# deepreinforce-ai/CUDA-L2

Measured on AMD Instinct MI355X. Metric: HGEMM TFLOP/s, higher is better.
Workload: dtype f16

## Files before the change

cuda-l2_amd/build.py:

```python
from __future__ import annotations

import concurrent.futures as cf
import hashlib
import os
import shutil
import subprocess
import sys
from pathlib import Path

PKG_DIR = Path(__file__).resolve().parent
REPO_DIR = PKG_DIR.parent
CSRC = PKG_DIR / "csrc"
INCLUDE = REPO_DIR / "include"
BUILD = PKG_DIR / "build"
OBJ = BUILD / "obj"
_SUFFIX = os.environ.get("HGEMM_LIB_SUFFIX", "")
LIB_DIR = PKG_DIR / ("lib_" + _SUFFIX if _SUFFIX else "lib")
BIN_DIR = PKG_DIR / "bin"
ROCM = Path(os.environ.get("ROCM_PATH", "/opt/rocm"))
HIPCC = str(ROCM / "bin" / "hipcc")
ARCH = "gfx950"

LIB_SOURCES = [
    "hgemm_inst_g0.hip",
    "hgemm_inst_g1.hip",
    "hgemm_inst_g2.hip",
    "hgemm_inst_g3.hip",
    "hgemm_inst_g4.hip",
    "hgemm_inst_g5.hip",
    "hgemm_inst_g6.hip",
    "hgemm_inst_g7.hip",
    "hgemm_inst_g8.hip",
    "hgemm_inst_g9.hip",
    "hgemm_inst_g10.hip",
    "hgemm_inst_g11.hip",
    "hgemm_inst_g12.hip",
    "hgemm_inst_g13.hip",
    "hgemm_inst_g14.hip",
    "hgemm_inst_g15.hip",
    "hgemm_inst_g16.hip",
    "hgemm_inst_g17.hip",
    "hgemm_registry.hip",
    "hgemm_plan.hip",
    "hgemm_api.hip",
    "hgemm_baselines.hip",
]

HIP_FLAGS = os.environ.get("HGEMM_EXTRA_HIPFLAGS", "").split() + [f"--offload-arch={ARCH}", "-O3", "-std=c++17", "-fPIC", "-Wall", "-Wno-unused-function",
             "-Wno-unused-result", "-Wno-unused-value", "-DROCBLAS_NO_DEPRECATED_WARNINGS", "-D__HIP_PLATFORM_AMD__"]


def _headers_digest() -> str:
    h = hashlib.sha256()
    for d in (CSRC, INCLUDE):
        for p in sorted(d.rglob("*")):
            if p.suffix in (".hpp", ".h", ".def", ".inc"):
                h.update(p.name.encode())
                h.update(p.read_bytes())
    return h.hexdigest()


def _run(cmd: list[str], verbose: bool) -> None:
    if verbose:
        print(" ".join(cmd), flush=True)
    res = subprocess.run(cmd, capture_output=True, text=True)
    if res.returncode != 0:
        sys.stderr.write(res.stdout + res.stderr)
        raise RuntimeError(f"build step failed ({res.returncode}): {' '.join(cmd)}")
    if verbose and (res.stdout or res.stderr):
        print(res.stdout + res.stderr, flush=True)


def compile_object(src: Path, extra_flags: list[str], hdr_digest: str, verbose: bool = False) -> Path:
    OBJ.mkdir(parents=True, exist_ok=True)
    cmd_core = [HIPCC, *HIP_FLAGS, *extra_flags, f"-I{CSRC}", f"-I{INCLUDE}", "-c"]
    key = hashlib.sha256()
    key.update(" ".join(cmd_core).encode())
    key.update(hdr_digest.encode())
    key.update(src.read_bytes())
    obj = OBJ / f"{src.stem}-{key.hexdigest()[:20]}.o"
    if not obj.exists():
        tmp = obj.with_suffix(f".tmp{os.getpid()}.o")
        _run([*cmd_core, str(src), "-o", str(tmp)], verbose)
        os.replace(tmp, obj)
    return obj


def build_library(verbose: bool = False, jobs: int | None = None) -> Path:
    hdr = _headers_digest()
    jobs = jobs or min(8, os.cpu_count() or 1)
    srcs = [CSRC / s for s in LIB_SOURCES]
    with cf.ThreadPoolExecutor(max_workers=jobs) as ex:
        objs = list(ex.map(lambda s: compile_object(s, [], hdr, verbose), srcs))
    LIB_DIR.mkdir(exist_ok=True)
    lib = LIB_DIR / "libhgemm_mi355x.so"
    stamp = LIB_DIR / ".libhgemm_mi355x.stamp"
    want = hashlib.sha256(" ".join(o.name for o in objs).encode()).hexdigest()
    if lib.exists() and stamp.exists() and stamp.read_text() == want:
        return lib
    tmp = lib.with_suffix(f".tmp{os.getpid()}.so")
    _run([HIPCC, f"--offload-arch={ARCH}", "-shared", "-fPIC", *map(str, objs), "-o", str(tmp),
          f"-L{ROCM / 'lib'}", "-lrocblas", "-lhipblaslt", "-lamdhip64",
          "-Wl,--no-undefined", "-Wl,-soname,libhgemm_mi355x.so"], verbose)
    os.replace(tmp, lib)
    stamp.write_text(want)
    return lib


def build_tools(verbose: bool = False) -> list[Path]:
    lib = build_library(verbose)
    hdr = _headers_digest()
    BIN_DIR.mkdir(exist_ok=True)
    out = []
    for name in ("hgemm_tune",):
        src = CSRC / "tools" / f"{name}.cpp"
        if not src.exists():
            continue
        obj = compile_object(src, ["-x", "hip"], hdr, verbose)
        exe = BIN_DIR / name
        stamp = BIN_DIR / f".{name}.stamp"
        want = obj.name + lib.name + str(lib.stat().st_mtime_ns)
        if not (exe.exists() and stamp.exists() and stamp.read_text() == want):
            _run([HIPCC, f"--offload-arch={ARCH}", str(obj), "-o", str(exe), f"-L{LIB_DIR}", "-lhgemm_mi355x",
                  f"-L{ROCM / 'lib'}", "-lamdhip64", "-lrocm_smi64", "-Wl,-rpath,$ORIGIN/../lib", f"-Wl,-rpath,{ROCM / 'lib'}"],
# ... 61 lines not shown
```

cuda-l2_amd/csrc/hgemm_api.hip:

```cpp
#include "hgemm_plan.hpp"
#include "hgemm_kernel_nn.hpp"
#include "hgemm_act.hpp"
#include "../../include/hgemm_mi355x.h"

#include <algorithm>
#include <atomic>
#include <cmath>
#include <cstdint>
#include <cstdlib>
#include <cstring>
#include <mutex>
#include <vector>

using namespace hgemm_mi355x;

namespace {

thread_local int g_last_hip_error = 0;
#ifdef HGEMM_ABLATION
int g_debug_flags = 0;
#endif
#ifdef HGEMM_TIMELINE
unsigned long long* g_timeline = nullptr;
int g_timeline_slots = 0;
// ... 734 lines not shown
  g_ws.clear();
  g_ws_retired.clear();
  return rc;
}

int hgemm_mi355x_release_stream_workspace(void* stream) {
  int dev = 0;
  if (hipGetDevice(&dev) != hipSuccess) return HGEMM_ERR_HIP;
  std::lock_guard<std::mutex> lk(g_ws_mutex);
  for (size_t i = 0; i < g_ws.size(); ++i) {
    if (g_ws[i].device != dev || g_ws[i].stream != (hipStream_t)stream) continue;
    int rc = HGEMM_OK;
    if (g_ws[i].ptr) {
      if (g_ws[i].captured) g_ws_retired.push_back(g_ws[i].ptr);
      else if (hipFree(g_ws[i].ptr) != hipSuccess) rc = HGEMM_ERR_HIP;
    }
    g_ws.erase(g_ws.begin() + (long)i);
    return rc;
  }
  return HGEMM_OK;
}

int hgemm_mi355x_reserve_workspace(int M, int N, int K, void* stream) {
  if (M <= 0 || N <= 0 || K <= 0) return HGEMM_ERR_BAD_ARG;
  int cfg = 0, splits = 1, group = 1;
  const int st = hgemm_mi355x_plan(M, N, K, &cfg, &splits, &group);
  if (st != HGEMM_OK) return st;
  const size_t ws = std::max(hgemm_mi355x_plan_workspace_bytes(cfg, splits, M, N, K), kCounterBytes + (size_t)256 * 256 * 256 * sizeof(float));
  float* slabs = nullptr; unsigned* counters = nullptr;
  const int rc = ensure_workspace(ws - kCounterBytes, (hipStream_t)stream, &slabs, &counters);
  return rc == HGEMM_ERR_NO_WORKSPACE_INTERNAL ? HGEMM_ERR_NO_WORKSPACE : rc;
}

int hgemm_mi355x_launch(int config_id, int splits_arg, int group_m, const void* a, const void* b,
                        const void* b_col_major, void* c, int M, int N, int K, int lda, int ldb,
                        int ldc, void* stream) {
  DisarmTiming disarm_timing;
  if (!a || !c || M <= 0 || N <= 0 || K <= 0) return HGEMM_ERR_BAD_ARG;
  if (config_id >= g_num_kernels || config_id < HGEMM_CONFIG_RAGGED) return HGEMM_ERR_BAD_ARG;
#ifdef HGEMM_TIMELINE
  ++g_timeline_count;
#endif
  hipStream_t s = (hipStream_t)stream;
  const bool aligned = mfma_path_ok(a, b_col_major, c, M, N, K, lda, ldb, ldc);
  unsigned ruled_out = 0;
  auto resolve = [&] {
    return resolve_launch(config_id, splits_arg, group_m, b != nullptr, b_col_major != nullptr, aligned, M, N, K, lda, ldb, ldc, ruled_out);
  };
  LaunchPlan p = resolve();
  float* slabs = nullptr; unsigned* counters = nullptr;
  while (p.status == HGEMM_OK && p.slab_bytes) {
    const int st = ensure_workspace(p.slab_bytes, s, &slabs, &counters);
    if (st == HGEMM_OK) break;
    if (st != HGEMM_ERR_NO_WORKSPACE_INTERNAL && p.form != FORM_HYBRID) return st;
    ruled_out |= 1u << p.form;
    p = resolve();
  }
  if (p.status != HGEMM_OK) return p.status;
  for (int i = 0; i < p.n; ++i) {
    GemmArgs& g = p.d[i].g;
    g.A = (const f16*)a; g.Bt = (const f16*)b_col_major; g.C = (f16*)c;
    if (p.d[i].epi != EPI_C16) {
      g.partial = slabs;
      if (p.counters) g.counters = counters;
    }
    const TimingSlot ts = timing_slot(p.d[i].start, p.d[i].stop);
    switch (p.d[i].thunk) {
      case THUNK_ENTRY: g_kernel_table[config_id].launch(g, p.d[i].grid, s, p.d[i].epi, ts); break;
      case THUNK_SPLITK_REDUCE: launch_splitk_reduce(g.partial, g.C, M, N, ldc, g.splits, s, ts); break;
      case THUNK_TAIL_REDUCE: launch_tail_reduce(g, g_kernel_table[config_id].bm, g_kernel_table[config_id].bn, s, ts); break;
      case THUNK_RAGGED: launch_ragged(g, s, ts); break;
      case THUNK_GENERIC: launch_generic((const f16*)a, (const f16*)b, (f16*)c, M, N, K, lda, N, ldc, s, ts); break;
    }
  }
  hipError_t err = hipGetLastError();
  if (err != hipSuccess) { g_last_hip_error = (int)err; return HGEMM_ERR_HIP; }
  return HGEMM_OK;
}

int hgemm_mi355x_set_one_item_kernel(int on) { return sq_one_set_enabled(on); }

unsigned long long hgemm_mi355x_one_item_kernel_launches(void) { return sq_one_launch_count(); }

int hgemm_mi355x_one_item_kernel_takes(int config_id, int splits, int group_m, int M, int N, int K, int lda, int ldb, int ldc) {
  if (M <= 0 || N <= 0 || K <= 0 || config_id >= g_num_kernels || config_id < HGEMM_CONFIG_RAGGED) return HGEMM_ERR_BAD_ARG;
  const LaunchPlan p = resolve_launch(config_id, splits, group_m, false, true, true, M, N, K, lda, ldb, ldc, 0);
  if (p.status != HGEMM_OK) return p.status;
  static const int q256 = hgemm_mi355x_config_by_name("q256x256_w2x2");
  if (config_id != q256) return 0;
  for (int i = 0; i < p.n; ++i)
    if (p.d[i].thunk == THUNK_ENTRY && sq_one_takes(p.d[i].g, p.d[i].grid, p.d[i].epi)) return 1;
  return 0;
}

int hgemm_mi355x_set_insitu(int enable) {
  const int old = insitu_enabled() ? 1 : 0;
  g_insitu_mode.store(enable ? 1 : 0);
  if (!enable) {
    std::lock_guard<std::mutex> lk(g_insitu_mutex);
    g_insitu.clear();
    g_insitu_epoch.fetch_add(1, std::memory_order_release);
  }
  return old;
}

int hgemm_mi355x_insitu_enabled(void) { return insitu_enabled() ? 1 : 0; }

int hgemm_mi355x_insitu_candidates(int M, int N, int K, int config_id[3], int splits[3], int group_m[3]) {
  if (M <= 0 || N <= 0 || K <= 0 || !config_id || !splits || !group_m) return 0;
  PlanTriple c[3];
  const int n = insitu_candidates(M, N, K, c);
  for (int i = 0; i < n; ++i) { config_id[i] = c[i].cfg; splits[i] = c[i].splits; group_m[i] = c[i].group_m; }
  return n;
}

int hgemm_mi355x_insitu_choice(int M, int N, int K, int* config_id, int* splits, int* group_m) {
  PlanTriple p;
  int dev = 0;
  if (hipGetDevice(&dev) != hipSuccess) { (void)hipGetLastError(); dev = 0; }
  if (!config_id || !splits || !group_m || !insitu_lookup(dev, M, N, K, &p)) return 0;
  *config_id = p.cfg; *splits = p.splits; *group_m = p.group_m;
  return 1;
}

int hgemm_mi355x_fp32(const void* a, const void* b, const void* bt, void* c, int M, int N, int K,
                      void* stream) {
  return run(HGEMM_ACC_FP32, a, b, bt, c, M, N, K, stream);
}

int hgemm_mi355x_fp16(const void* a, const void* b, const void* bt, void* c, int M, int N, int K,
                      void* stream) {
  return run(HGEMM_ACC_FP16, a, b, bt, c, M, N, K, stream);
}

int hgemm_mi355x_nn_num_configs(void) { return kLayoutNN.t.count; }
const char* hgemm_mi355x_nn_config_name(int id) { return tr_config_name(kLayoutNN, id); }
int hgemm_mi355x_nn_config_by_name(const char* name) { return tr_config_by_name(kLayoutNN, name); }
int hgemm_mi355x_nn_config_info(int id, int out[8]) { return tr_config_info(kLayoutNN, id, out); }
int hgemm_mi355x_nn_plan(int M, int N, int K, int* nn_config, int* splits) { return tr_plan(kLayoutNN, M, N, K, nn_config, splits); }
int hgemm_mi355x_nn_runs(int nn_config, int M, int N, int K, int lda, int ldb, int ldc) { return tr_runs(kLayoutNN, TR_F16, kOutC16, nn_config, M, N, K, lda, ldb, ldc); }
size_t hgemm_mi355x_nn_plan_workspace_bytes(int nn_config, int splits, int M, int N, int K) {
  return tr_plan_workspace_bytes(kLayoutNN, nn_config, splits, M, N, K);
}
int hgemm_mi355x_nn_reserve_workspace(int M, int N, int K, void* stream) { return tr_reserve_workspace(kLayoutNN, M, N, K, stream); }
int hgemm_mi355x_launch_nn(int nn_config, int splits_arg, const void* a, const void* b, void* c, int M, int N, int K, int lda, int ldb,
                           int ldc, void* stream) {
  return tr_launch(kLayoutNN, TR_F16, kOutC16, nn_config, splits_arg, a, b, nullptr, c, M, N, K, lda, ldb, ldc, stream);
}
int hgemm_mi355x_nn_fp32(const void* a, const void* b, void* c, int M, int N, int K, void* stream) { return tr_run(kLayoutNN, TR_F16, kOutC16, a, b, nullptr, c, M, N, K, stream); }
int hgemm_mi355x_nn_fp16(const void* a, const void* b, void* c, int M, int N, int K, void* stream) { return tr_run(kLayoutNN, TR_F16, kOutC16, a, b, nullptr, c, M, N, K, stream); }
int hgemm_mi355x_selfcheck_launch_nn(int nn_config, int splits, int operands, int M, int N, int K, int lda, int ldb, int ldc, int ruled_out,
                                     long long out[20]) {
  return tr_selfcheck_launch(kLayoutNN, TR_F16, kOutC16, nn_config, splits, operands, M, N, K, lda, ldb, ldc, ruled_out, out);
}

int hgemm_mi355x_ta_num_configs(void) { return kLayoutTA.t.count; }
const char* hgemm_mi355x_ta_config_name(int id) { return tr_config_name(kLayoutTA, id); }
int hgemm_mi355x_ta_config_by_name(const char* name) { return tr_config_by_name(kLayoutTA, name); }
int hgemm_mi355x_ta_config_info(int id, int out[8]) { return tr_config_info(kLayoutTA, id, out); }
int hgemm_mi355x_ta_plan(int M, int N, int K, int* ta_config, int* splits) { return tr_plan(kLayoutTA, M, N, K, ta_config, splits); }
int hgemm_mi355x_ta_runs(int ta_config, int M, int N, int K, int lda, int ldb, int ldc) { return tr_runs(kLayoutTA, TR_F16, kOutC16, ta_config, M, N, K, lda, ldb, ldc); }
size_t hgemm_mi355x_ta_plan_workspace_bytes(int ta_config, int splits, int M, int N, int K) {
  return tr_plan_workspace_bytes(kLayoutTA, ta_config, splits, M, N, K);
}
int hgemm_mi355x_ta_reserve_workspace(int M, int N, int K, void* stream) { return tr_reserve_workspace(kLayoutTA, M, N, K, stream); }
int hgemm_mi355x_launch_ta(int ta_config, int splits_arg, const void* a_col_major, const void* b, void* c, int M, int N, int K, int lda,
                           int ldb, int ldc, void* stream) {
  return tr_launch(kLayoutTA, TR_F16, kOutC16, ta_config, splits_arg, a_col_major, b, nullptr, c, M, N, K, lda, ldb, ldc, stream);
}
int hgemm_mi355x_ta_fp32(const void* a_col_major, const void* b, void* c, int M, int N, int K, void* stream) { return tr_run(kLayoutTA, TR_F16, kOutC16, a_col_major, b, nullptr, c, M, N, K, stream); }
int hgemm_mi355x_ta_fp16(const void* a_col_major, const void* b, void* c, int M, int N, int K, void* stream) { return tr_run(kLayoutTA, TR_F16, kOutC16, a_col_major, b, nullptr, c, M, N, K, stream); }
int hgemm_mi355x_selfcheck_launch_ta(int ta_config, int splits, int operands, int M, int N, int K, int lda, int ldb, int ldc, int ruled_out,
                                     long long out[20]) {
  return tr_selfcheck_launch(kLayoutTA, TR_F16, kOutC16, ta_config, splits, operands, M, N, K, lda, ldb, ldc, ruled_out, out);
}
// ... 304 lines not shown
```

cuda-l2_amd/csrc/hgemm_inst_g13.hip:

```cpp
#include "hgemm_launch.hpp"
#include "hgemm_kernel_sq_one.hpp"

#include <atomic>

namespace hgemm_mi355x {

template __global__ void hgemm_tn_sq_one_kernel<CfgSQOne>(const GemmArgs);

namespace {
#ifdef HGEMM_TIMELINE
std::atomic<int> g_sq_one_on{0};
#else
std::atomic<int> g_sq_one_on{1};
#endif
std::atomic<unsigned long long> g_sq_one_launches{0};
}

int sq_one_set_enabled(int on) { return g_sq_one_on.exchange(on ? 1 : 0); }
unsigned long long sq_one_launch_count() { return g_sq_one_launches.load(); }

bool sq_one_takes(const GemmArgs& g, int grid, int epi) {
  if (!g_sq_one_on.load(std::memory_order_relaxed)) return false;
  if (epi != EPI_C16 || !c_takes_wide_stores(g)) return false;
  if (g.K % (BK * CfgSQOne::KT) != 0 || g.K / BK < SQ_ONE_MIN_STEPS) return false;
  if (g.splits != 1 || g.tail_tiles != 0 || g.items > grid) return false;
  if (g.flags & (ARG_XCD_STAGGER | ARG_PHASE_OFFSET | ARG_PHASE_OFFSET4)) return false;
#ifdef HGEMM_ABLATION
  if (g.debug) return false;
#endif
  return true;
}

bool launch_sq_one(const GemmArgs& g, int grid, hipStream_t stream, int epi, TimingSlot ts) {
  if (!sq_one_takes(g, grid, epi)) return false;
  g_sq_one_launches.fetch_add(1, std::memory_order_relaxed);
  HGEMM_LAUNCH((hgemm_tn_sq_one_kernel<CfgSQOne>), grid, CfgSQOne::THREADS, stream, ts, g);
  return true;
}

}
```

cuda-l2_amd/csrc/hgemm_launch.hpp:

```cpp
#pragma once
#include "hgemm_kernel_rs.hpp"
#include "hgemm_kernel_sq.hpp"
#include "hgemm_kernel_wd.hpp"
#include "hgemm_kernel_lu.hpp"

#include <hip/hip_ext.h>

#include <type_traits>

namespace hgemm_mi355x {

struct LaunchTiming { hipEvent_t start = nullptr, stop = nullptr; };
extern thread_local LaunchTiming t_launch_timing;

struct TimingSlot { hipEvent_t start = nullptr, stop = nullptr; };
inline TimingSlot timing_slot(bool first, bool last) {
  TimingSlot s;
  if (first) { s.start = t_launch_timing.start; t_launch_timing.start = nullptr; }
  if (last) { s.stop = t_launch_timing.stop; t_launch_timing.stop = nullptr; }
  return s;
}

#define HGEMM_LAUNCH(KERNEL, GRID, THREADS, STREAM, SLOT, ...)                                              \
  do {                                                                                                      \
    if ((SLOT).start || (SLOT).stop)                                                                        \
      hipExtLaunchKernelGGL(KERNEL, dim3(GRID), dim3(THREADS), 0, STREAM, (SLOT).start, (SLOT).stop, 0,     \
                            __VA_ARGS__);                                                                   \
    else                                                                                                    \
      hipLaunchKernelGGL(KERNEL, dim3(GRID), dim3(THREADS), 0, STREAM, __VA_ARGS__);                        \
  } while (0)

template <class CFG>
void launch_cfg(const GemmArgs& g, int grid, hipStream_t stream, int epi, TimingSlot ts) {
  if (epi == EPI_STREAMK) {
    if constexpr (CFG::BM * CFG::BN <= 256 * 128) HGEMM_LAUNCH((hgemm_tn_sk_kernel<CFG>), grid, CFG::THREADS, stream, ts, g);
  } else if (epi == EPI_FUSED)
    HGEMM_LAUNCH((hgemm_tn_kernel<CFG, EPI_FUSED>), grid, CFG::THREADS, stream, ts, g);
  else if (epi == EPI_SLAB)
    HGEMM_LAUNCH((hgemm_tn_kernel<CFG, EPI_SLAB>), grid, CFG::THREADS, stream, ts, g);
  else
    HGEMM_LAUNCH((hgemm_tn_kernel<CFG, EPI_C16>), grid, CFG::THREADS, stream, ts, g);
}

inline bool c_takes_wide_stores(const GemmArgs& g) {
  return ((g.N & 7) == 0) && ((g.ldc & 7) == 0) && ((reinterpret_cast<uintptr_t>(g.C) & 15) == 0);
}

template <class CFG>
void launch_sp(const GemmArgs& g, int grid, hipStream_t stream, int epi, TimingSlot ts) {
  const bool wide = c_takes_wide_stores(g);
  if (epi == EPI_FUSED)
    HGEMM_LAUNCH((hgemm_tn_sp_kernel<CFG, SP_EPI_FUSED>), grid, CFG::THREADS, stream, ts, g);
  else if (epi == EPI_SLAB)
    HGEMM_LAUNCH((hgemm_tn_sp_kernel<CFG, SP_EPI_SLAB>), grid, CFG::THREADS, stream, ts, g);
  else if (wide)
    HGEMM_LAUNCH((hgemm_tn_sp_kernel<CFG, SP_EPI_WIDE>), grid, CFG::THREADS, stream, ts, g);
  else
    HGEMM_LAUNCH((hgemm_tn_sp_kernel<CFG, SP_EPI_NARROW>), grid, CFG::THREADS, stream, ts, g);
}

template <class CFG, int FLAG>
void launch_sq_variant(const GemmArgs& g, int grid, hipStream_t stream, int epi, TimingSlot ts) {
  const bool wide = c_takes_wide_stores(g);
  if (epi == EPI_FUSED)
    HGEMM_LAUNCH((hgemm_tn_sq_kernel<CFG, SP_EPI_FUSED | FLAG>), grid, CFG::THREADS, stream, ts, g);
  else if (epi == EPI_SLAB)
    HGEMM_LAUNCH((hgemm_tn_sq_kernel<CFG, SP_EPI_SLAB | FLAG>), grid, CFG::THREADS, stream, ts, g);
  else if (wide)
    HGEMM_LAUNCH((hgemm_tn_sq_kernel<CFG, SP_EPI_WIDE | FLAG>), grid, CFG::THREADS, stream, ts, g);
  else
    HGEMM_LAUNCH((hgemm_tn_sq_kernel<CFG, SP_EPI_NARROW | FLAG>), grid, CFG::THREADS, stream, ts, g);
}

bool launch_sq_one(const GemmArgs& g, int grid, hipStream_t stream, int epi, TimingSlot ts);
bool sq_one_takes(const GemmArgs& g, int grid, int epi);
int sq_one_set_enabled(int on);
unsigned long long sq_one_launch_count();

template <class CFG>
void launch_sq(const GemmArgs& g, int grid, hipStream_t stream, int epi, TimingSlot ts) {
  if constexpr (std::is_same_v<CFG, CfgSQOne>) {
    if (launch_sq_one(g, grid, stream, epi, ts)) return;
  }
  if constexpr (CFG::MI == 16) {
    if (g.K % (BK * CFG::KT) != 0) return launch_sq_variant<CFG, EPI_KTAIL>(g, grid, stream, epi, ts);
    if (g.flags & ARG_XCD_STAGGER) return launch_sq_variant<CFG, EPI_KSTAGGER>(g, grid, stream, epi, ts);
  }
  launch_sq_variant<CFG, 0>(g, grid, stream, epi, ts);
}

template <class CFG, int FLAG>
void launch_rs_variant(const GemmArgs& g, int grid, hipStream_t stream, int epi, TimingSlot ts) {
  if (epi == EPI_FUSED)
    HGEMM_LAUNCH((hgemm_tn_rs_kernel<CFG, EPI_FUSED | FLAG>), grid, CFG::THREADS, stream, ts, g);
  else if (epi == EPI_SLAB)
    HGEMM_LAUNCH((hgemm_tn_rs_kernel<CFG, EPI_SLAB | FLAG>), grid, CFG::THREADS, stream, ts, g);
  else
    HGEMM_LAUNCH((hgemm_tn_rs_kernel<CFG, EPI_C16 | FLAG>), grid, CFG::THREADS, stream, ts, g);
}

template <class CFG>
void launch_rs(const GemmArgs& g, int grid, hipStream_t stream, int epi, TimingSlot ts) {
  if (epi == EPI_STREAMK)
    HGEMM_LAUNCH((hgemm_tn_rs_sk_kernel<CFG>), grid, CFG::THREADS, stream, ts, g);
  else if (g.K % CFG::BKS != 0)
    launch_rs_variant<CFG, EPI_KTAIL>(g, grid, stream, epi, ts);
  else
    launch_rs_variant<CFG, 0>(g, grid, stream, epi, ts);
}

template <class CFG>
void launch_wd(const GemmArgs& g, int grid, hipStream_t stream, int epi, TimingSlot ts) {
  if (epi == EPI_FUSED)
    HGEMM_LAUNCH((hgemm_tn_wd_kernel<CFG, EPI_FUSED>), grid, CFG::THREADS, stream, ts, g);
  else if (epi == EPI_SLAB)
    HGEMM_LAUNCH((hgemm_tn_wd_kernel<CFG, EPI_SLAB>), grid, CFG::THREADS, stream, ts, g);
  else
    HGEMM_LAUNCH((hgemm_tn_wd_kernel<CFG, EPI_C16>), grid, CFG::THREADS, stream, ts, g);
}

template <class CFG>
void launch_lu(const GemmArgs& g, int grid, hipStream_t stream, int epi, TimingSlot ts) {
  if (epi == EPI_SLAB)
    HGEMM_LAUNCH((hgemm_tn_lu_kernel<CFG, EPI_SLAB>), grid, CFG::THREADS, stream, ts, g);
  else
    HGEMM_LAUNCH((hgemm_tn_lu_kernel<CFG, EPI_C16>), grid, CFG::THREADS, stream, ts, g);
}

enum class Family : char { T = 't', S = 's', Q = 'q', R = 'r', W = 'w', U = 'u' };
enum class KTail : char { NONE, PADDED, DIRECT };

struct KernelEntry {
  const char* name;
  Family family;
  int bm, bn, wm, wn, mi, nbuf;
  int threads, lds_bytes;
  void (*launch)(const GemmArgs&, int, hipStream_t, int, TimingSlot);
  int persistent_wgs;
  bool has_fused;
  int kgran;
  KTail ktail;
  int sk_wgs_per_cu;
  bool explicit_only;
};
inline bool w_splits_k(const KernelEntry& e) { return e.family == Family::W && e.wm * e.wn == 1; }

extern const KernelEntry g_kernel_table[];
extern const int g_num_kernels;

void launch_splitk_reduce(const float* partial, f16* C, int M, int N, int ldc, int splits,
                          hipStream_t stream, TimingSlot ts);
void launch_tail_reduce(const GemmArgs& g, int BM, int BN, hipStream_t stream, TimingSlot ts);
void launch_ragged(const GemmArgs& g, hipStream_t stream, TimingSlot ts);
void launch_generic(const f16* A, const f16* B, f16* C, int M, int N, int K, int lda, int ldb,
                    int ldc, hipStream_t stream, TimingSlot ts);

}
```

include/hgemm_mi355x.h:

```cpp
#ifndef HGEMM_MI355X_H_
#define HGEMM_MI355X_H_

#include <stddef.h>

#ifdef __cplusplus
extern "C" {
#endif

typedef enum {
  HGEMM_OK = 0,
  HGEMM_ERR_BAD_ARG = -1,
  HGEMM_ERR_TOO_LARGE = -2,
  HGEMM_ERR_HIP = -3,
  HGEMM_ERR_BACKEND = -4,
  HGEMM_ERR_NOT_READY = -5,
  HGEMM_ERR_NO_ALGO = -6,
  HGEMM_ERR_NO_WORKSPACE = -7
} hgemm_status_t;

typedef enum { HGEMM_ACC_FP32 = 0, HGEMM_ACC_FP16 = 1 } hgemm_acc_t;

#define HGEMM_CONFIG_GENERIC (-1)
#define HGEMM_CONFIG_RAGGED  (-2)

// ... 97 lines not shown
int bgemm_mi355x_tn_num_configs(void);
const char* bgemm_mi355x_tn_config_name(int tn_config);
int bgemm_mi355x_tn_config_by_name(const char* name);
int bgemm_mi355x_tn_config_info(int tn_config, int out[8]);
int bgemm_mi355x_tn_plan(int M, int N, int K, int* tn_config, int* splits);
size_t bgemm_mi355x_tn_plan_workspace_bytes(int tn_config, int splits, int M, int N, int K);
int bgemm_mi355x_tn_reserve_workspace(int M, int N, int K, void* stream);

int bgemm_mi355x_tn_bias(const void* a, const void* b_col_major, const void* bias, void* c, int M, int N, int K, void* stream);
int bgemm_mi355x_launch_tn_bias(int tn_config, int splits, const void* a, const void* b_col_major, const void* bias, void* c,
                                int M, int N, int K, int lda, int ldb, int ldc, void* stream);
int bgemm_mi355x_tn_bias_runs(int tn_config, int M, int N, int K, int lda, int ldb, int ldc);

#define HGEMM_ACT_RELU 1
#define HGEMM_ACT_GELU 2
#define HGEMM_ACT_GELU_TANH 3
int bgemm_mi355x_tn_bias_act(const void* a, const void* b_col_major, const void* bias, void* c, int M, int N, int K, int act, void* stream);
int bgemm_mi355x_launch_tn_bias_act(int tn_config, int splits, const void* a, const void* b_col_major, const void* bias, void* c,
                                    int M, int N, int K, int lda, int ldb, int ldc, int act, void* stream);
int bgemm_mi355x_tn_bias_act_runs(int tn_config, int M, int N, int K, int lda, int ldb, int ldc);

int bgemm_mi355x_tn_bias_act_aux(const void* a, const void* b_col_major, const void* bias, void* c, void* z_out, int M, int N, int K, int act,
                                 void* stream);
int bgemm_mi355x_launch_tn_bias_act_aux(int tn_config, int splits, const void* a, const void* b_col_major, const void* bias, void* c,
                                        void* z_out, int M, int N, int K, int lda, int ldb, int ldc, int ldz, int act, void* stream);
int bgemm_mi355x_tn_bias_act_aux_runs(int tn_config, int M, int N, int K, int lda, int ldb, int ldc, int ldz);

int bgemm_mi355x_nn_dact(const void* a, const void* b, const void* z, void* c, int M, int N, int K, int act, void* stream);
int bgemm_mi355x_launch_nn_dact(int nn_config, int splits, const void* a, const void* b, const void* z, void* c, int M, int N, int K,
                                int lda, int ldb, int ldc, int ldz, int act, void* stream);
int bgemm_mi355x_nn_dact_runs(int nn_config, int M, int N, int K, int lda, int ldb, int ldc, int ldz);

int bgemm_mi355x_nn_dact_dbias(const void* a, const void* b, const void* z, void* c, float* db32, int M, int N, int K, int act,
                               int accumulate, void* stream);
int bgemm_mi355x_launch_nn_dact_dbias(int nn_config, int splits, const void* a, const void* b, const void* z, void* c, float* db32, int M,
                                      int N, int K, int lda, int ldb, int ldc, int ldz, int act, int accumulate, void* stream);
int bgemm_mi355x_nn_dact_dbias_runs(int nn_config, int M, int N, int K, int lda, int ldb, int ldc, int ldz);
size_t bgemm_mi355x_nn_dact_dbias_plan_workspace_bytes(int nn_config, int splits, int M, int N, int K);
int bgemm_mi355x_nn_dact_dbias_reserve_workspace(int M, int N, int K, void* stream);

int bgemm_mi355x_colsum_c32(const void* x, float* out32, int M, int N, int ldx, int accumulate, void* stream);

const char* hgemm_mi355x_strerror(int status);
int hgemm_mi355x_last_hip_error(void);
const char* hgemm_mi355x_version(void);

int hgemm_rocblas_init(void);
int hgemm_rocblas_destroy(void);
int hgemm_rocblas_nn(const void* a, const void* b, void* c, int M, int N, int K, int acc, void* stream);
int hgemm_rocblas_tn(const void* a, const void* b_col_major, void* c, int M, int N, int K, int acc, void* stream);
int hgemm_rocblas_ta(const void* a_col_major, const void* b, void* c, int M, int N, int K, int acc, void* stream);
int bgemm_rocblas_nn(const void* a, const void* b, void* c, int M, int N, int K, void* stream);
int bgemm_rocblas_ta(const void* a_col_major, const void* b, void* c, int M, int N, int K, void* stream);
int bgemm_rocblas_tn(const void* a, const void* b_col_major, void* c, int M, int N, int K, void* stream);

int hgemm_hipblaslt_heuristic_init(void);
int hgemm_hipblaslt_heuristic_destroy(void);
int hgemm_hipblaslt_heuristic_nn(const void* a, const void* b, void* c, int M, int N, int K, int acc, void* stream);
int hgemm_hipblaslt_heuristic_tn(const void* a, const void* b_col_major, void* c, int M, int N, int K, int acc, void* stream);

int hgemm_hipblaslt_autotune_init(void);
int hgemm_hipblaslt_autotune_destroy(void);
int hgemm_hipblaslt_autotune_find_best_nn(int M, int N, int K, int acc);
int hgemm_hipblaslt_autotune_find_best_tn(int M, int N, int K, int acc);
int hgemm_hipblaslt_autotune_nn(const void* a, const void* b, void* c, int M, int N, int K, int acc, void* stream);
int hgemm_hipblaslt_autotune_tn(const void* a, const void* b_col_major, void* c, int M, int N, int K, int acc, void* stream);
int hgemm_hipblaslt_autotune_set_cache(const char* path);
int hgemm_hipblaslt_autotune_from_cache(int tn);
int hgemm_hipblaslt_autotune_cache_stats(int* hits, int* misses);
int hgemm_hipblaslt_autotune_candidates(int tn);
double hgemm_hipblaslt_autotune_best_ms(int tn);
int hgemm_hipblaslt_compute16_fallback(int which, int tn);

int hgemm_fill_normal_f16(void* device_ptr, size_t n, unsigned long long seed, void* stream);

void* hgemm_mi355x_event_create(void);
int hgemm_mi355x_event_destroy(void* event);
int hgemm_mi355x_time_next_launch(void* start_event, void* stop_event);
double hgemm_mi355x_event_elapsed_us(void* start_event, void* stop_event);

int hgemm_mi355x_set_one_item_kernel(int on);
unsigned long long hgemm_mi355x_one_item_kernel_launches(void);
int hgemm_mi355x_one_item_kernel_takes(int config_id, int splits, int group_m, int M, int N, int K, int lda, int ldb, int ldc);

#ifdef __cplusplus
}
#endif
#endif
```

Baseline: 1418.

## Add one-item sq kernel variant overlapping epilogue stores with final K-step MFMAs

Adds a new kernel for the q256x256 one-workgroup-per-CU path that statically schedules the epilogue (accumulator reads, f16 conversion, LDS staging writes/reads and global buffer stores) into the MFMA slots of the last two K steps. A constexpr plan interleaves fragment reads, waitcnts and paced stores so the epilogue is hidden behind the tail compute instead of running after it. It is enabled by default when K has enough steps and replaces the existing one-item kernel launch. This adds a large hand-scheduled inline-asm body with a risk of register pressure or wrong waitcnt placement.

```diff
diff --git a/cuda-l2_amd/build.py b/cuda-l2_amd/build.py
--- a/cuda-l2_amd/build.py
+++ b/cuda-l2_amd/build.py
@@ -40,6 +40,7 @@
     "hgemm_inst_g15.hip",
     "hgemm_inst_g16.hip",
     "hgemm_inst_g17.hip",
+    "hgemm_inst_g18.hip",
     "hgemm_registry.hip",
     "hgemm_plan.hip",
     "hgemm_api.hip",
diff --git a/cuda-l2_amd/csrc/hgemm_api.hip b/cuda-l2_amd/csrc/hgemm_api.hip
--- a/cuda-l2_amd/csrc/hgemm_api.hip
+++ b/cuda-l2_amd/csrc/hgemm_api.hip
@@ -840,15 +840,27 @@
 
 unsigned long long hgemm_mi355x_one_item_kernel_launches(void) { return sq_one_launch_count(); }
 
-int hgemm_mi355x_one_item_kernel_takes(int config_id, int splits, int group_m, int M, int N, int K, int lda, int ldb, int ldc) {
+static int one_item_takes(bool tail, int config_id, int splits, int group_m, int M, int N, int K, int lda, int ldb, int ldc) {
   if (M <= 0 || N <= 0 || K <= 0 || config_id >= g_num_kernels || config_id < HGEMM_CONFIG_RAGGED) return HGEMM_ERR_BAD_ARG;
   const LaunchPlan p = resolve_launch(config_id, splits, group_m, false, true, true, M, N, K, lda, ldb, ldc, 0);
   if (p.status != HGEMM_OK) return p.status;
   static const int q256 = hgemm_mi355x_config_by_name("q256x256_w2x2");
   if (config_id != q256) return 0;
   for (int i = 0; i < p.n; ++i)
-    if (p.d[i].thunk == THUNK_ENTRY && sq_one_takes(p.d[i].g, p.d[i].grid, p.d[i].epi)) return 1;
+    if (p.d[i].thunk == THUNK_ENTRY && sq_one_takes(p.d[i].g, p.d[i].grid, p.d[i].epi) && (!tail || sq_tail_takes(p.d[i].g))) return 1;
   return 0;
+}
+
+int hgemm_mi355x_one_item_kernel_takes(int config_id, int splits, int group_m, int M, int N, int K, int lda, int ldb, int ldc) {
+  return one_item_takes(false, config_id, splits, group_m, M, N, K, lda, ldb, ldc);
+}
+
+int hgemm_mi355x_set_one_item_tail(int on) { return sq_tail_set_enabled(on); }
+
+unsigned long long hgemm_mi355x_one_item_tail_launches(void) { return sq_tail_launch_count(); }
+
+int hgemm_mi355x_one_item_tail_takes(int config_id, int splits, int group_m, int M, int N, int K, int lda, int ldb, int ldc) {
+  return one_item_takes(true, config_id, splits, group_m, M, N, K, lda, ldb, ldc);
 }
 
 int hgemm_mi355x_set_insitu(int enable) {
diff --git a/cuda-l2_amd/csrc/hgemm_inst_g13.hip b/cuda-l2_amd/csrc/hgemm_inst_g13.hip
--- a/cuda-l2_amd/csrc/hgemm_inst_g13.hip
+++ b/cuda-l2_amd/csrc/hgemm_inst_g13.hip
@@ -34,6 +34,7 @@
 bool launch_sq_one(const GemmArgs& g, int grid, hipStream_t stream, int epi, TimingSlot ts) {
   if (!sq_one_takes(g, grid, epi)) return false;
   g_sq_one_launches.fetch_add(1, std::memory_order_relaxed);
+  if (launch_sq_tail(g, grid, stream, ts)) return true;
   HGEMM_LAUNCH((hgemm_tn_sq_one_kernel<CfgSQOne>), grid, CfgSQOne::THREADS, stream, ts, g);
   return true;
 }
diff --git a/cuda-l2_amd/csrc/hgemm_inst_g18.hip b/cuda-l2_amd/csrc/hgemm_inst_g18.hip
--- /dev/null
+++ b/cuda-l2_amd/csrc/hgemm_inst_g18.hip
@@ -0,0 +1,33 @@
+#include "hgemm_launch.hpp"
+#include "hgemm_kernel_sq_tail.hpp"
+
+#include <atomic>
+
+namespace hgemm_mi355x {
+
+template __global__ void hgemm_tn_sq_tail_kernel<CfgSQOne>(const GemmArgs);
+
+namespace {
+#ifdef HGEMM_TIMELINE
+std::atomic<int> g_sq_tail_on{0};
+#else
+std::atomic<int> g_sq_tail_on{1};
+#endif
+std::atomic<unsigned long long> g_sq_tail_launches{0};
+}
+
+int sq_tail_set_enabled(int on) { return g_sq_tail_on.exchange(on ? 1 : 0); }
+unsigned long long sq_tail_launch_count() { return g_sq_tail_launches.load(); }
+
+bool sq_tail_takes(const GemmArgs& g) {
+  return g_sq_tail_on.load(std::memory_order_relaxed) && g.K / BK >= SQ_TAIL_MIN_STEPS;
+}
+
+bool launch_sq_tail(const GemmArgs& g, int grid, hipStream_t stream, TimingSlot ts) {
+  if (!sq_tail_takes(g)) return false;
+  g_sq_tail_launches.fetch_add(1, std::memory_order_relaxed);
+  HGEMM_LAUNCH((hgemm_tn_sq_tail_kernel<CfgSQOne>), grid, CfgSQOne::THREADS, stream, ts, g);
+  return true;
+}
+
+}
diff --git a/cuda-l2_amd/csrc/hgemm_kernel_sq_tail.hpp b/cuda-l2_amd/csrc/hgemm_kernel_sq_tail.hpp
--- /dev/null
+++ b/cuda-l2_amd/csrc/hgemm_kernel_sq_tail.hpp
@@ -0,0 +1,386 @@
+#pragma once
+
+#include "hgemm_kernel_sq_one.hpp"
+
+#ifndef HGEMM_SQ_TAIL_PACE
+#define HGEMM_SQ_TAIL_PACE 8
+#endif
+#ifndef HGEMM_SQ_TAIL_LEAD
+#define HGEMM_SQ_TAIL_LEAD 4
+#endif
+
+namespace hgemm_mi355x {
+
+constexpr int SQ_TAIL_DEPTH = 2;
+constexpr int SQ_TAIL_MIN_STEPS = SQ_ONE_MIN_STEPS + (SQ_TAIL_DEPTH - 1);
+
+template <int LEAD_, int PACE_>
+struct SqTailPlan {
+  static constexpr int FM = 8, FN = 8, NG = FN / 4, GROUPS = FM * NG, NM = 4 * FM * FN, LEAD = LEAD_, PACE = PACE_;
+  static constexpr int SY = 16 * LEAD - 24;
+  static constexpr int NOPS = 14 + 16 * GROUPS;
+  static constexpr int ACC_DIST = 3;
+  static constexpr int RD_AHEAD = 12;
+  static_assert(LEAD >= 3 && LEAD <= FM && PACE >= 1, "the sync point sits behind the slice-1 B reads of tile nk-2");
+  enum { OP_NONE, OP_VA, OP_VB, OP_W, OP_R, OP_S };
+  signed char mi[NM], mj[NM], mt[NM], ms[NM];
+  short fin[FM];
+  short first1[FM];
+  short frag[NM], fgap[40];
+  short eop[NM], egap[NOPS];
+  unsigned char ds[NM];
+  short lw[NM + 1], lwlast[NM + 1];
+  short lwfirst[NM + 1];
+  short sw[NOPS];
+  int n_gap_ops;
+
+  static constexpr int op_kind(int e) {
+    if (e < 12) return e % 3 == 0 ? OP_VA : e % 3 == 1 ? OP_VB : OP_W;
+    if (e < 14) return OP_R;
+    const int k = (e - 14) / 16, r = (e - 14) % 16;
+    if (r == 12 || r == 15) return OP_S;
+    if (k + 1 >= GROUPS) return OP_NONE;
+    if (r < 12) return r % 3 == 0 ? OP_VA : r % 3 == 1 ? OP_VB : OP_W;
+    return OP_R;
+  }
+  static constexpr int op_group(int e) {
+    if (e < 14) return 0;
+    const int k = (e - 14) / 16, r = (e - 14) % 16;
+    return (r == 12 || r == 15) ? k : k + 1;
+  }
+  static constexpr int op_sub(int e) {
+    if (e < 12) return e / 3;
+    if (e < 14) return e - 12;
+    const int r = (e - 14) % 16;
+    return r < 12 ? r / 3 : r == 12 ? 0 : r == 15 ? 1 : r - 13;
+  }
+
+  constexpr SqTailPlan()
+      : mi(), mj(), mt(), ms(), fin(), first1(), frag(), fgap(), eop(), egap(), ds(), lw(), lwlast(), lwfirst(), sw(), n_gap_ops(0) {
+    int n = 0;
+    auto run = [&](int i, int t, int s) {
+      for (int j = 0; j < FN; ++j, ++n) { mi[n] = (signed char)i; mj[n] = (signed char)j; mt[n] = (signed char)t; ms[n] = (signed char)s; }
+    };
+    run(0, 0, 0); run(1, 0, 0); run(0, 0, 1); run(1, 0, 1);
+    for (int i = 2; i < LEAD; ++i) { run(i, 0, 0); run(i, 0, 1); }
+    for (int i = 0; i < LEAD; ++i) { first1[i] = (short)n; run(i, 1, 0); run(i, 1, 1); fin[i] = (short)(n - 1); }
+    for (int i = LEAD; i < FM; ++i) { run(i, 0, 0); run(i, 0, 1); first1[i] = (short)n; run(i, 1, 0); run(i, 1, 1); fin[i] = (short)(n - 1); }
+    for (int g = 0; g < NM; ++g) { frag[g] = -1; eop[g] = -1; ds[g] = 0; }
+    for (int g = 0; g <= NM; ++g) { lw[g] = -1; lwlast[g] = -1; lwfirst[g] = -1; }
+    for (int e = 0; e < NOPS; ++e) { egap[e] = -1; sw[e] = 0; }
+    auto put = [&](int id, int g) { frag[g] = (short)id; fgap[id] = (short)g; ds[g] = 1; };
+    for (int j = 0; j < FN; ++j) put(j, j);
+    int g = SY;
+    for (int j = 0; j < FN; ++j) put(8 + j, g++);
+    put(24, g++);
+    for (int j = 0; j < FN; ++j) put(16 + j, g++);
+    put(32, g++); put(25, g++); put(33, g++);
+    for (int i = 2; i < FM; ++i) { put(24 + i, first1[i] - RD_AHEAD); put(32 + i, first1[i] - RD_AHEAD + 1); }
+    int cur = 0, last_store = -PACE;
+    bool open = true;
+    for (int e = 0; e < NOPS; ++e) {
+      const int kind = op_kind(e);
+      if (kind == OP_NONE) { if (open) n_gap_ops = e + 1; continue; }
+      if (!open) continue;
+      int at = cur;
+      const int avail = fin[op_group(e) / NG] + ACC_DIST;
+      if (kind != OP_S && at < avail) at = avail;
+      if (kind == OP_S && at < last_store + PACE) at = last_store + PACE;
+      while (at < NM - 1 && frag[at] >= 0) ++at;
+      if (at >= NM - 1) { open = false; continue; }
+      eop[at] = (short)e; egap[e] = (short)at; cur = at + 1;
+      if (kind == OP_W || kind == OP_R) ds[at] = 1;
+      if (kind == OP_S) last_store = at;
+      n_gap_ops = e + 1;
+    }
+    auto younger = [&](int gap_of_read, int slot) { int c = 0; for (int x = gap_of_read + 1; x < slot; ++x) c += ds[x]; return c; };
+    auto wait_at = [&](int slot, int first_id, int last_id) {
+      lw[slot] = (short)younger(fgap[last_id], slot); lwfirst[slot] = (short)first_id; lwlast[slot] = (short)last_id;
+    };
+    wait_at(16, 0, 7);
+    wait_at(first1[0], 8, 24);
+    wait_at(first1[0] + FN, 16, 33);
+    for (int i = 2; i < FM; ++i) wait_at(first1[i], 24 + i, 32 + i);
+    for (int e = 0; e < n_gap_ops; ++e)
+      if (op_kind(e) == OP_S && op_sub(e) == 0 && egap[e] >= 0) {
+        int r = -1;
+        for (int x = 0; x < e; ++x) if (op_kind(x) == OP_R && op_group(x) == op_group(e) && op_sub(x) == 1) r = x;
+        sw[e] = (short)younger(egap[r], egap[e]);
+      }
+  }
+  constexpr bool ok() const {
+    for (int i = 2; i < FM; ++i) if (first1[i] - RD_AHEAD <= SY + 2 * FN + 4) return false;
+    if (SY < FN + 2 || SY + 2 * FN + 4 > first1[0] - 2) return false;
+    for (int e = 0; e < n_gap_ops; ++e) if (op_kind(e) != OP_NONE && egap[e] < 0) return false;
+    return true;
+  }
+};
+
+#if defined(__HIP_DEVICE_COMPILE__)
+struct SqTailRegs {
+  f16x8 X[8], Z[8], U[8], V[8], Y[8], W[8], P[8], Q[8];
+  unsigned vB0h1, vB1h0, vB1h1, vA1h0, vA1h1;
+  unsigned waddr[4], raddr, voff[2], row8;
+  __amdgpu_buffer_rsrc_t rsC;
+  bool nt;
+  unsigned lo, hi;
+  __attribute__((ext_vector_type(4))) unsigned rb[2][2];
+};
+
+template <int ID>
+__device__ __forceinline__ void sq_tail_read_frag(SqTailRegs& c) {
+  constexpr int r = ID % 8;
+  f16x8& dst = ID < 8 ? c.V[r] : ID < 16 ? c.Y[r] : ID < 24 ? c.W[r] : ID < 32 ? c.P[r] : c.Q[r];
+  const unsigned a = ID < 8 ? c.vB0h1 : ID < 16 ? c.vB1h0 : ID < 24 ? c.vB1h1 : ID < 32 ? c.vA1h0 : c.vA1h1;
+  asm volatile("ds_read_b128 %0, %1 offset:%2" : "=v"(dst) : "v"(a), "n"(r * 16 * ROW_BYTES) : "memory");
+}
+template <int CNT, int FIRST, int LAST>
+__device__ __forceinline__ void sq_tail_wait(SqTailRegs& c) {
+#define SQT8(A) "+v"(c.A[0]), "+v"(c.A[1]), "+v"(c.A[2]), "+v"(c.A[3]), "+v"(c.A[4]), "+v"(c.A[5]), "+v"(c.A[6]), "+v"(c.A[7])
+  if constexpr (FIRST == 0) asm volatile("s_waitcnt lgkmcnt(%8)" : SQT8(V) : "n"(CNT) : "memory");
+  else if constexpr (FIRST == 8) asm volatile("s_waitcnt lgkmcnt(%9)" : SQT8(Y), "+v"(c.P[0]) : "n"(CNT) : "memory");
+  else if constexpr (FIRST == 16) asm volatile("s_waitcnt lgkmcnt(%11)" : SQT8(W), "+v"(c.Q[0]), "+v"(c.P[1]), "+v"(c.Q[1]) : "n"(CNT) : "memory");
+  else asm volatile("s_waitcnt lgkmcnt(%2)" : "+v"(c.P[FIRST - 24]), "+v"(c.Q[LAST - 32]) : "n"(CNT) : "memory");
+#undef SQT8
+}
+
+template <class PLAN, int E, bool GAP>
+__device__ __forceinline__ void sq_tail_op(SqTailRegs& c) {
+  constexpr PLAN tab{};
+  constexpr int kind = PLAN::op_kind(E), k = PLAN::op_group(E), sub = PLAN::op_sub(E);
+  constexpr int i = k / PLAN::NG, gg = k % PLAN::NG, b = k & 1;
+  if constexpr (kind == PLAN::OP_VA || kind == PLAN::OP_VB) {
+    constexpr int a0 = (i * PLAN::FN + gg * 4 + sub) * 4 + (kind == PLAN::OP_VB ? 2 : 0);
+    unsigned t;
+    if constexpr (kind == PLAN::OP_VA)
+      asm volatile("v_accvgpr_read_b32 %0, a[%2]\n\tv_accvgpr_read_b32 %1, a[%3]\n\tv_cvt_pk_f16_f32 %0, %0, %1" : "=&v"(c.lo), "=&v"(t) : "n"(a0), "n"(a0 + 1));
+    else
+      asm volatile("v_accvgpr_read_b32 %0, a[%2]\n\tv_accvgpr_read_b32 %1, a[%3]\n\tv_cvt_pk_f16_f32 %0, %0, %1" : "=&v"(c.hi), "=&v"(t) : "n"(a0), "n"(a0 + 1));
+  } else if constexpr (kind == PLAN::OP_W) {
+    const __attribute__((ext_vector_type(2))) unsigned pk = {c.lo, c.hi};
+    asm volatile("ds_write_b64 %0, %1 offset:%2" ::"v"(c.waddr[sub]), "v"(pk), "n"(b * 2048) : "memory");
+  } else if constexpr (kind == PLAN::OP_R) {
+    asm volatile("ds_read_b128 %0, %1 offset:%2" : "=v"(c.rb[b][sub]) : "v"(c.raddr), "n"(b * 2048 + sub * 1024) : "memory");
+  } else if constexpr (kind == PLAN::OP_S) {
+    if constexpr (sub == 0)
+      asm volatile("s_waitcnt lgkmcnt(%2)" : "+v"(c.rb[b][0]), "+v"(c.rb[b][1]) : "n"(GAP ? (int)tab.sw[E] : 0) : "memory");
+    const unsigned soff = (unsigned)(i * 2 + sub) * c.row8;
+    if (c.nt) asm volatile("buffer_store_dwordx4 %0, %1, %2, %3 offen nt\n\ts_nop 1" ::"v"(c.rb[b][sub]), "v"(c.voff[gg]), "s"(c.rsC), "s"(soff) : "memory");
+    else      asm volatile("buffer_store_dwordx4 %0, %1, %2, %3 offen\n\ts_nop 1" ::"v"(c.rb[b][sub]), "v"(c.voff[gg]), "s"(c.rsC), "s"(soff) : "memory");
+  }
+}
+
+template <class PLAN, int N>
+__device__ __forceinline__ void sq_tail_slot(SqTailRegs& c) {
+  constexpr PLAN tab{};
+  constexpr int i = tab.mi[N], j = tab.mj[N], t = tab.mt[N], s = tab.ms[N];
+  if constexpr (N == PLAN::SY) sp_sync();
+  if constexpr (tab.lw[N] >= 0) sq_tail_wait<tab.lw[N], tab.lwfirst[N], tab.lwlast[N]>(c);
+  const f16x8& a = t == 0 ? (s == 0 ? c.X[i] : c.Z[i]) : (s == 0 ? c.P[i] : c.Q[i]);
+  const f16x8& bb = t == 0 ? (s == 0 ? c.U[j] : c.V[j]) : (s == 0 ? c.Y[j] : c.W[j]);
+  sp_mfma(i * PLAN::FN + j, bb, a);
+  if constexpr (tab.frag[N] >= 0) sq_tail_read_frag<tab.frag[N]>(c);
+  if constexpr (tab.eop[N] >= 0) sq_tail_op<PLAN, tab.eop[N], true>(c);
+  if constexpr (N == PLAN::SY - 2) wait_vmcnt<0>();
+}
+template <class PLAN, int... N>
+__device__ __forceinline__ void sq_tail_slots(SqTailRegs& c, std::integer_sequence<int, N...>) { (sq_tail_slot<PLAN, N>(c), ...); }
+template <class PLAN, int E0, int... E>
+__device__ __forceinline__ void sq_tail_remainder(SqTailRegs& c, std::integer_sequence<int, E...>) { (sq_tail_op<PLAN, E0 + E, false>(c), ...); }
+#endif
+
+#define SQ1_FRAG(STAGE, OPOFF, H) ((STAGE) + (OPOFF) + foff[H])
+#define SQ1_K_STEP(YS, ZS, LA, EB, LB, EA, VMP, VMQ, NEXT)                                                              \
+  do {                                                                                                                  \
+    char* st  = smem + (step & 1) * CFG::STAGE_BYTES;                                                                   \
+    char* nst = smem + ((step + 1) & 1) * CFG::STAGE_BYTES;                                                             \
+    sq_interval<CFG, 0, LA, EB, VMP, NEXT>(fX, fU, fV, SQ1_FRAG(st, b_base_off, 1), SQ1_FRAG(st, b_base_off, 1),        \
+                                           ZS, SQ1_FRAG(nst, a_base_off, 1), SQ1_FRAG(nst, a_base_off, 1), wave, voffA, voffB, \
+                                           rsA, st, kbA, rsB, st, kbB);                                                 \
+    kbA += ROW_BYTES;                                                                                                   \
+    sq_interval<CFG, 1, LB, EA, VMQ, NEXT>(YS, fV, fX, SQ1_FRAG(nst, a_base_off, 0), SQ1_FRAG(nst, a_base_off, 0),      \
+                                           fU, SQ1_FRAG(nst, b_base_off, 0), SQ1_FRAG(nst, b_base_off, 0), wave, voffA, voffB, \
+                                           rsB, st, kbB, rsA, nst, kbA);                                                \
+    kbB += ROW_BYTES;                                                                                                   \
+    ++step;                                                                                                             \
+  } while (0)
+#define SQ1_FULL_STEP(YS, ZS) SQ1_K_STEP(YS, ZS, true, true, true, true, CFG::NJA + CFG::NJB, CFG::NJA + CFG::NJB, true)
+
+template <class CFG>
+__global__ void __launch_bounds__(CFG::THREADS) hgemm_tn_sq_tail_kernel(const GemmArgs g) {
+  prefetch_kernargs<sizeof(GemmArgs)>();
+#if defined(__HIP_DEVICE_COMPILE__)
+  static_assert(CFG::MI == 16 && CFG::KT == 1 && CFG::WGS == 1, "the 16x16x32, K = 64 per stage, one-workgroup-per-CU member");
+  static_assert(sp_staged_ok<CFG>(CFG::LDS_BYTES), "the LDS-staged wide epilogue");
+  using PLAN = SqTailPlan<HGEMM_SQ_TAIL_LEAD, HGEMM_SQ_TAIL_PACE>;
+  static_assert(CFG::FM == PLAN::FM && CFG::FN == PLAN::FN && PLAN{}.ok(), "the tail's plan is q256x256_w2x2's");
+  constexpr int BM = CFG::BM, BN = CFG::BN, FM = CFG::FM, FN = CFG::FN, MI = CFG::MI;
+  constexpr int NFA = CFG::NFA, NFB = CFG::NFB;
+#ifdef HGEMM_TIMELINE
+  constexpr int TL_EXTRA = 64;
+#else
+  constexpr int TL_EXTRA = 0;
+#endif
+  constexpr int STAGED_BYTES = CFG::NW * SP_STAGED_BYTES_PER_WAVE;
+  __shared__ __attribute__((aligned(1024))) char smem[CFG::LDS_BYTES + 64 + STAGED_BYTES + TL_EXTRA];
+
+  const int tid  = threadIdx.x;
+  HGEMM_TL_STAMP(smem + CFG::LDS_BYTES, 0, tid);
+  HGEMM_TL_REALTIME(smem + CFG::LDS_BYTES, 1, tid);
+  const int lane = tid & 63;
+  const int wave = __builtin_amdgcn_readfirstlane(tid >> 6);
+  const int wave_m = wave / CFG::WN;
+  const int wave_n = wave % CFG::WN;
+
+  const ItemWalk walk = persistent_walk(g.items);
+  if (walk.count == 0) return;
+  const TileCoord tc = map_logical(g, walk.base + walk.first, BM, BN);
+  const int m0 = __builtin_amdgcn_readfirstlane(tc.m0), n0 = __builtin_amdgcn_readfirstlane(tc.n0);
+  const int nk = __builtin_amdgcn_readfirstlane(tc.nk);
+
+  const int lr = lane & (MI - 1), lq = lane / MI, sw = (lr >> 1) & 7;
+  int foff[2];
+#pragma unroll
+  for (int h = 0; h < 2; ++h) foff[h] = lr * ROW_BYTES + (((h * 4 + lq) ^ sw) << 4);
+  const int a_base_off = wave_m * CFG::TM * ROW_BYTES;
+  const int b_base_off = BM * ROW_BYTES + wave_n * CFG::TN * ROW_BYTES;
+
+  sp_reserve_agprs<CFG::AGPRS>();
+
+  static_assert(CFG::NW % 2 == 0, "the swizzle key of a wave's row blocks must not depend on the piece");
+  const uint32_t chunk0 = (uint32_t)((lane & 7) ^ (((wave & 1) << 2) | (lane >> 4)));
+  uint32_t voffA[CFG::PA], voffB[CFG::PB];
+#pragma unroll
+  for (int q = 0; q < CFG::PA; ++q) voffA[q] = ((uint32_t)((wave + q * CFG::NW) * 8 + (lane >> 3)) * (uint32_t)g.lda + chunk0 * 8u) * 2u;
+#pragma unroll
+  for (int q = 0; q < CFG::PB; ++q) voffB[q] = ((uint32_t)((wave + q * CFG::NW) * 8 + (lane >> 3)) * (uint32_t)g.ldb + chunk0 * 8u) * 2u;
+  auto tile_rsrc = [](const f16* base, int row0, int rows, int ld) __attribute__((always_inline)) {
+    const uintptr_t addr = reinterpret_cast<uintptr_t>(base + (size_t)row0 * ld);
+    const uintptr_t uni = ((uintptr_t)(uint32_t)__builtin_amdgcn_readfirstlane((int)(addr >> 32)) << 32) |
+                          (uint32_t)__builtin_amdgcn_readfirstlane((int)(uint32_t)addr);
+    const unsigned long long rem = (unsigned long long)(rows - row0) * (unsigned long long)ld * 2ull;
+    const unsigned range = (unsigned)__builtin_amdgcn_readfirstlane((int)(rem > 0xFFFFFFFFull ? 0xFFFFFFFFu : (unsigned)rem));
+    return __builtin_amdgcn_make_buffer_rsrc((void*)uni, 0, (int)range, 0x00020000);
+  };
+  const __amdgpu_buffer_rsrc_t rsA = tile_rsrc(g.A, m0, g.M, g.lda), rsB = tile_rsrc(g.Bt, n0, g.N, g.ldb);
+  const uint32_t kb0 = (uint32_t)__builtin_amdgcn_readfirstlane(tc.k_begin * 2);
+  HGEMM_TL_STAMP(smem + CFG::LDS_BYTES + 64 + STAGED_BYTES, 0, tid);
+  constexpr int NZ = FM * FN, NPIECE = 2 * (CFG::NJA + CFG::NJB);
+  int zi = 0, pi = 0;
+#pragma unroll
+  for (int s = 0; s < 2; ++s) {
+#pragma unroll
+    for (int p = 0; p < CFG::NJA; ++p) {
+      sq_issue_piece<CFG, 0>(rsA, voffA, smem + s * CFG::STAGE_BYTES, wave, p, kb0 + s * ROW_BYTES);
+      for (++pi; zi < (pi * NZ) / NPIECE; ++zi) sp_zero_acc(zi);
+    }
+#pragma unroll
+    for (int p = 0; p < CFG::NJB; ++p) {
+      sq_issue_piece<CFG, 1>(rsB, voffB, smem + s * CFG::STAGE_BYTES, wave, p, kb0 + s * ROW_BYTES);
+      for (++pi; zi < (pi * NZ) / NPIECE; ++zi) sp_zero_acc(zi);
+    }
+  }
+  __builtin_amdgcn_sched_barrier(0);
+#pragma unroll
+  for (; zi < NZ; ++zi) sp_zero_acc(zi);
+  HGEMM_TL_STAMP(smem + CFG::LDS_BYTES + 64 + STAGED_BYTES, 1, tid);
+  wait_vmcnt<CFG::NJA + CFG::NJB>();
+  __builtin_amdgcn_s_barrier();
+  HGEMM_TL_STAMP(smem + CFG::LDS_BYTES + 64 + STAGED_BYTES, 2, tid);
+
+  f16x8 fX[NFA], fY[NFA], fZ[NFA], fU[NFB], fV[NFB];
+#pragma unroll
+  for (int r = 0; r < NFA; ++r) {
+    fX[r] = *(const f16x8*)(SQ1_FRAG(smem, a_base_off, 0) + r * MI * ROW_BYTES);
+    fY[r] = *(const f16x8*)(SQ1_FRAG(smem, a_base_off, 1) + r * MI * ROW_BYTES);
+  }
+#pragma unroll
+  for (int r = 0; r < NFB; ++r) fU[r] = *(const f16x8*)(SQ1_FRAG(smem, b_base_off, 0) + r * MI * ROW_BYTES);
+  uint32_t kbA = kb0 + 2 * ROW_BYTES, kbB = kb0 + 2 * ROW_BYTES;
+  __builtin_amdgcn_sched_barrier(0);
+  __builtin_amdgcn_s_waitcnt(kWaitLgkm0);
+  sp_sync();
+#pragma unroll
+  for (int p = 0; p < CFG::DA; ++p) sq_issue_piece<CFG, 0>(rsA, voffA, smem, wave, p, kbA);
+
+  int step = 0;
+  HGEMM_TL_STAMP(smem + CFG::LDS_BYTES, 2, tid);
+  HGEMM_TL_STAMP(smem + CFG::LDS_BYTES, 3, tid);
+  if ((nk & 1) == 0) {
+    sq_settle(fX, fY, fU);
+    SQ1_FULL_STEP(fY, fZ);
+#pragma unroll
+    for (int r = 0; r < NFA; ++r) fY[r] = fZ[r];
+  }
+  sq_settle(fX, fY, fU);
+#pragma clang loop unroll(disable)
+  for (int t = step; t + 4 < nk; t += 2) {
+    SQ1_FULL_STEP(fY, fZ);
+    SQ1_FULL_STEP(fZ, fY);
+  }
+  sq_settle(fX, fY, fU);
+  SQ1_K_STEP(fY, fZ, true, true, true, false, CFG::NJA + CFG::NJB, CFG::NJA + CFG::NJB, true);
+
+  SqTailRegs c;
+  {
+    int ln;
+    asm volatile("v_mbcnt_lo_u32_b32 %0, -1, 0\n\tv_mbcnt_hi_u32_b32 %0, -1, %0" : "=v"(ln));
+    char* stage = smem + CFG::LDS_BYTES + 64 + wave * SP_STAGED_BYTES_PER_WAVE;
+    const unsigned lds0 = (unsigned)(uintptr_t)(__attribute__((address_space(3))) char*)stage;
+    const int wrow = ln & 15, wq = ln >> 4;
+#pragma unroll
+    for (int jj = 0; jj < 4; ++jj) c.waddr[jj] = lds0 + wrow * 128 + (((jj * 2 + (wq >> 1)) ^ (wrow & 7)) << 4) + (wq & 1) * 8;
+    const int rrow = ln >> 3, rch = ln & 7;
+    c.raddr = lds0 + rrow * 128 + ((rch ^ (rrow & 7)) << 4);
+    const int m_wave = m0 + wave_m * CFG::TM, n_wave = n0 + wave_n * CFG::TN;
+    const uintptr_t caddr = reinterpret_cast<uintptr_t>(g.C + (size_t)m_wave * g.ldc + n_wave);
+    const uintptr_t cuni = ((uintptr_t)(uint32_t)__builtin_amdgcn_readfirstlane((int)(caddr >> 32)) << 32) |
+                           (uint32_t)__builtin_amdgcn_readfirstlane((int)(uint32_t)caddr);
+    const long long rem = ((long long)(g.M - m_wave) * g.ldc - n_wave) * 2;
+    const unsigned range = __builtin_amdgcn_readfirstlane((int)(rem <= 0 ? 0 : rem > 0x7FFFFFFFLL ? 0x7FFFFFFF : rem));
+    c.rsC = __builtin_amdgcn_make_buffer_rsrc((void*)cuni, 0, (int)range, 0x00020000);
+#pragma unroll
+    for (int gg = 0; gg < PLAN::NG; ++gg)
+      c.voff[gg] = (n_wave + gg * 64 + rch * 8 < g.N) ? (unsigned)(rrow * g.ldc + gg * 64 + rch * 8) * 2u : 0x80000000u;
+    c.row8 = (unsigned)__builtin_amdgcn_readfirstlane((int)((unsigned)g.ldc * 16u));
+    c.nt = (g.flags & ARG_NT_STORE) != 0;
+    const unsigned s0 = (unsigned)(uintptr_t)(lds_void_t*)(smem + (step & 1) * CFG::STAGE_BYTES);
+    const unsigned s1 = (unsigned)(uintptr_t)(lds_void_t*)(smem + ((step + 1) & 1) * CFG::STAGE_BYTES);
+    c.vB0h1 = s0 + b_base_off + foff[1];
+    c.vB1h0 = s1 + b_base_off + foff[0];
+    c.vB1h1 = s1 + b_base_off + foff[1];
+    c.vA1h0 = s1 + a_base_off + foff[0];
+    c.vA1h1 = s1 + a_base_off + foff[1];
+    unsigned ntw = c.nt ? 1u : 0u;
+    asm volatile("" : "+v"(c.waddr[0]), "+v"(c.waddr[1]), "+v"(c.waddr[2]), "+v"(c.waddr[3]), "+v"(c.raddr), "+v"(c.voff[0]), "+v"(c.voff[1]),
+                 "+v"(c.vB0h1), "+v"(c.vB1h0), "+v"(c.vB1h1), "+v"(c.vA1h0), "+v"(c.vA1h1), "+s"(c.row8), "+s"(ntw), "+s"(c.rsC));
+    c.nt = ntw != 0;
+  }
+#pragma unroll
+  for (int r = 0; r < 8; ++r) { c.X[r] = fX[r]; c.Z[r] = fZ[r]; c.U[r] = fU[r]; }
+  __builtin_amdgcn_sched_barrier(0);
+  __builtin_amdgcn_s_waitcnt(kWaitLgkm0);
+  sq_settle(c.X, c.Z, c.U);
+  sq_tail_slots<PLAN>(c, std::make_integer_sequence<int, PLAN::NM>{});
+  step += 2;
+  HGEMM_TL_STAMP(smem + CFG::LDS_BYTES, 4, tid);
+  sp_mfma_drain();
+  sq_tail_remainder<PLAN, PLAN{}.n_gap_ops>(c, std::make_integer_sequence<int, PLAN::NOPS - PLAN{}.n_gap_ops>{});
+  __builtin_amdgcn_sched_barrier(0);
+#ifdef HGEMM_TIMELINE
+  HGEMM_TL_STAMP(smem + CFG::LDS_BYTES, 5, tid);
+  wait_vmcnt<0>();
+  HGEMM_TL_STAMP(smem + CFG::LDS_BYTES, 6, tid);
+  HGEMM_TL_REALTIME(smem + CFG::LDS_BYTES, 7, tid);
+  sq_timeline_record(g, smem + CFG::LDS_BYTES, smem + CFG::LDS_BYTES + 64 + STAGED_BYTES, step, 1, tid);
+#endif
+#endif
+}
+
+#undef SQ1_FULL_STEP
+#undef SQ1_K_STEP
+#undef SQ1_FRAG
+
+extern template __global__ void hgemm_tn_sq_tail_kernel<CfgSQOne>(const GemmArgs);
+
+}
diff --git a/cuda-l2_amd/csrc/hgemm_launch.hpp b/cuda-l2_amd/csrc/hgemm_launch.hpp
--- a/cuda-l2_amd/csrc/hgemm_launch.hpp
+++ b/cuda-l2_amd/csrc/hgemm_launch.hpp
@@ -76,6 +76,10 @@
 bool sq_one_takes(const GemmArgs& g, int grid, int epi);
 int sq_one_set_enabled(int on);
 unsigned long long sq_one_launch_count();
+bool launch_sq_tail(const GemmArgs& g, int grid, hipStream_t stream, TimingSlot ts);
+bool sq_tail_takes(const GemmArgs& g);
+int sq_tail_set_enabled(int on);
+unsigned long long sq_tail_launch_count();
 
 template <class CFG>
 void launch_sq(const GemmArgs& g, int grid, hipStream_t stream, int epi, TimingSlot ts) {
diff --git a/include/hgemm_mi355x.h b/include/hgemm_mi355x.h
--- a/include/hgemm_mi355x.h
+++ b/include/hgemm_mi355x.h
@@ -203,6 +203,9 @@
 int hgemm_mi355x_set_one_item_kernel(int on);
 unsigned long long hgemm_mi355x_one_item_kernel_launches(void);
 int hgemm_mi355x_one_item_kernel_takes(int config_id, int splits, int group_m, int M, int N, int K, int lda, int ldb, int ldc);
+int hgemm_mi355x_set_one_item_tail(int on);
+unsigned long long hgemm_mi355x_one_item_tail_launches(void);
+int hgemm_mi355x_one_item_tail_takes(int config_id, int splits, int group_m, int M, int N, int K, int lda, int ldb, int ldc);
 
 #ifdef __cplusplus
 }
```

Result: no change. 1424, median of 6 (+0.4%).
